# KatiaJDL/CenterPoly

Measured on AMD Instinct MI355X. Metric: inference img/s @2048x1024 DLA-34 (1 GPU), higher is better.
Workload: dtype f32 I/O; split-bf16 x3 contraction (a*b ~ ah*bh + ah*bl + al*bh on bf16 MFMA, ~2^-16 per product) in the convolutions, the heads and DCNv2; f32 accumulate; 1 GPU; BASELINE config 2: DLA-34 + DCNv2, 1x3x1024x2048 synthetic, 16-vertex cartesian head, K=128, forward + sigmoid + NMS/top-k/decode; parallelism=single

## Files before the change

### centerpoly_amd/_C.py

```python
import ctypes
import os
from ctypes import POINTER, Structure, c_char_p, c_float, c_int32, c_int64, c_size_t, c_void_p

import torch

_HERE = os.path.dirname(os.path.abspath(__file__))
LIB_PATH = os.path.join(_HERE, "csrc", "libcenterpoly_hip.so")

CP_OK = 0
REP = {"cartesian": 0, "polar": 1, "polar_fixed": 2}
HEATMAP_UMICH, HEATMAP_ELLIPSE = 0, 1
L1_PLAIN, L1_POLAR, L1_POLAR_FIXED, L1_RELU20, L1_SMOOTH = 0, 1, 2, 3, 4
DCN_BWD_EXACT_F32, DCN_BWD_NARROW_TILES = 1, 2
DCN_CONTRACTION = {"f32": 0, "bf16x3": 1, "bf16x3_region": 3}


class DcnShape(Structure):
    _fields_ = [(n, c_int32) for n in ("B", "Cin", "H", "W", "Cout", "kh", "kw", "stride", "pad",
                                       "dil", "deformable_groups")]


class TargetShape(Structure):
    _fields_ = [(n, c_int32) for n in ("B", "max_objs", "nbr_points", "num_classes", "out_h", "out_w",
                                       "rep", "no_reorder_flip")]
# ... 62 lines not shown
                                        c_size_t, _P]),
    "cp_polygon_masks_workspace_bytes": (c_size_t, [c_int32, c_int32]),
    "cp_polygon_masks": (c_int32, [_P, _P, c_int32, c_int32, c_int32, _P, _P, _P, c_size_t, _P]),
    "cp_annot_rays_ids": (c_int32, [_P, c_int32, c_int32, _P, _P, c_int32, c_int32, _P, _P]),
    "cp_annot_rays_masks": (c_int32, [_P, c_int32, c_int32, _P, c_int32, c_int32, _P, _P]),
    "cp_polygon_paint_workspace_bytes": (c_size_t, [c_int32, c_int32]),
    "cp_polygon_paint": (c_int32, [_P, _P, _P, c_int32, c_int32, c_int32, c_int32, _P, _P, c_size_t, _P]),
    "cp_render_overlay_workspace_bytes": (c_size_t, [c_int32, c_int32]),
    "cp_render_overlay": (c_int32, [_P, c_int32, c_int32, _P, c_int32, c_int32, _P, _P, _P, _P, c_int32, _P, c_int32, _P,
                                    c_int32, _P, _P, _P, c_size_t, _P]),
    "cp_render_heatmap": (c_int32, [_P, c_int32, c_int32, c_int32, c_int32, _P, _P, _P, _P, c_int32, c_int32, _P, _P]),
    "cp_oracle_map": (c_int32, [_P, _P] + [c_int32] * 5 + [_P, _P]),
    "cp_id_histogram": (c_int32, [_P, c_int32, c_int32, _P, _P]),
    "cp_instance_overlaps_workspace_bytes": (c_size_t, [c_int32] * 4),
    "cp_instance_overlaps": (c_int32, [_P, c_int32, _P, c_int32, c_int32, _P, c_int32, _P, c_int32, _P, _P, _P, _P,
                                       c_size_t, _P]),
    "cp_polydet_post_process": (c_int32, [_P, _P, c_float, c_int32, c_int32, c_int32, _P, _P]),
    "cp_polydet_targets_workspace_bytes": (c_size_t, [POINTER(TargetShape)]),
    "cp_polydet_targets": (c_int32, [POINTER(TargetShape)] + [_P] * 19 + [_P, c_size_t, _P]),
    "cp_polydet_targets_ex": (c_int32, [POINTER(TargetShape), c_int32] + [_P] * 19 + [_P, c_size_t, _P]),
    "cp_polydet_dense_targets": (c_int32, [POINTER(TargetShape), _P, _P, c_size_t, _P, _P, _P]),
    "cp_conv_direct_supported": (c_int32, [c_int32] * 5),
    "cp_conv_direct_wgrad_supported": (c_int32, [c_int32] * 5),
    "cp_conv_direct_wgrad": (c_int32, [_P, _P, _P] + [c_int32] * 8 + [_P]),
    "cp_conv_direct_forward": (c_int32, [_P, _P, _P, _P] + [c_int32] * 9 + [_P]),
    "cp_conv_direct_forward_ex": (c_int32, [_P, _P, _P, _P] + [c_int32] * 10 + [_P]),
    "cp_conv3x3_mfma_supported": (c_int32, [c_int32] * 4),
    "cp_conv3x3_mfma_weight_bytes": (c_size_t, [c_int32] * 2),
    "cp_conv3x3_mfma_prepare": (c_int32, [_P, c_int32, c_int32, c_int32, _P, _P]),
    "cp_conv3x3_mfma_forward": (c_int32, [_P, _P, _P, _P, _P] + [c_int32] * 6 + [_P]),
    "cp_conv_mfma_weight_bytes": (c_size_t, [c_int32] * 3),
    "cp_conv_mfma_prepare": (c_int32, [_P, c_int32, c_int32, c_int32, c_int32, _P, _P]),
    "cp_conv3x3_s2_wgrad_supported": (c_int32, [c_int32] * 4),
    "cp_conv3x3_s2_wgrad": (c_int32, [_P, _P, _P] + [c_int32] * 5 + [_P]),
    "cp_conv7x7_c3_supported": (c_int32, [c_int32] * 4),
    "cp_conv7x7_c3_weight_bytes": (c_size_t, [c_int32]),
    "cp_conv7x7_c3_prepare": (c_int32, [_P, c_int32, _P, _P]),
    "cp_conv7x7_c3_forward": (c_int32, [_P, _P, _P, _P] + [c_int32] * 6 + [_P]),
    "cp_conv_mfma_prepare_blocks": (c_int32, [c_int32] * 3),
    "cp_conv_mfma_prepare_batch": (c_int32, [_P, c_int32, c_int32, _P]),
    "cp_conv_mfma_forward": (c_int32, [_P, _P, c_int32, _P, _P, _P, _P] + [c_int32] * 6 + [_P]),
    "cp_conv_mfma_forward_strided": (c_int32, [_P, _P, c_int32, _P, _P, _P, _P] + [c_int32] * 7 + [_P]),
    "cp_dla_base_pair_supported": (c_int32, [c_int32] * 2),
    "cp_dla_base_pair_forward": (c_int32, [_P] * 6 + [c_int32] * 3 + [_P]),
    "cp_conv_mfma_forward_split": (c_int32, [_P, c_int32, _P, _P, _P, _P] + [c_int32] * 9 + [_P]),
    "cp_activation_split": (c_int32, [_P, _P] + [c_int32] * 4 + [_P]),
    "cp_activation_unsplit": (c_int32, [_P, _P] + [c_int32] * 4 + [_P]),
    "cp_conv1x1_stream_supported": (c_int32, [_P, c_int32, c_int32, c_int32, c_int32]),
    "cp_conv1x1_stream_weight_bytes": (c_size_t, [c_int32] * 2),
    "cp_conv1x1_stream_prepare": (c_int32, [_P, c_int32, c_int32, _P, _P]),
    "cp_conv1x1_stream_forward": (c_int32, [_P, _P, c_int32, _P, _P, _P, _P] + [c_int32] * 5 + [_P]),
    "cp_conv1x1_stream_form": (c_int32, [c_int32] * 5),
    "cp_conv1x1_stream_forward_form": (c_int32, [_P, _P, c_int32, _P, _P, _P, _P] + [c_int32] * 7 + [_P]),
    "cp_conv_mfma_input_grad_relu_workspace_bytes": (c_size_t, [c_int32] * 4),
    "cp_conv_mfma_input_grad_relu": (c_int32, [_P] * 5 + [c_int32] * 6 + [_P, c_size_t, _P]),
    "cp_conv3x3_s2_input_grad": (c_int32, [_P, _P, _P, _P] + [c_int32] * 5 + [_P]),
    "cp_conv3x3_mfma_wgrad_supported": (c_int32, [c_int32] * 4),
    "cp_conv3x3_mfma_wgrad": (c_int32, [_P, _P, _P] + [c_int32] * 5 + [_P]),
    "cp_conv_mfma_wgrad": (c_int32, [_P, _P, _P] + [c_int32] * 6 + [_P]),
    "cp_heads_fused_w2_bytes": (c_size_t, [c_int32]),
    "cp_heads_fused_prepare_w2": (c_int32, [_P, c_int32, c_int32, _P, _P]),
    "cp_heads_fused_forward": (c_int32, [_P, _P, _P, _P, _P, _P, _P] + [c_int32] * 6 + [_P]),
    "cp_maxpool2x2_forward": (c_int32, [_P, _P] + [c_int32] * 4 + [_P]),
    "cp_maxpool2x2_backward": (c_int32, [_P, _P, _P] + [c_int32] * 4 + [_P]),
    "cp_conv1x1_act_forward": (c_int32, [_P, c_int64, _P, c_int32, _P, _P, _P, c_int32, c_int32, c_int32, c_int64, _P]),
    "cp_soft_nms": (c_int32, [_P, c_int32, c_int32, c_float, c_float, c_float, c_int32]),
    "cp_soft_nms_device": (c_int32, [_P, c_int32, _P, _P, c_int32, c_float, c_float, c_float, c_int32, _P, _P]),
    "cp_merge_detections_workspace_bytes": (c_size_t, [c_int32] * 4),
    "cp_merge_detections": (c_int32, [_P] + [c_int32] * 6 + [c_float] * 3 + [c_int32, _P, _P, _P, c_size_t, _P]),
    "cp_polydet_decode_workspace_bytes": (c_size_t, [c_int32] * 5),
    "cp_polydet_decode": (c_int32, [_P, _P, _P, _P] + [c_int32] * 7 + [_P, _P, _P, _P, c_size_t, _P]),
    "cp_polydet_decode_ex": (c_int32, [_P, _P, _P, _P] + [c_int32] * 8 + [_P, _P, _P, _P, c_size_t, _P]),
    "cp_sigmoid_focal_workspace_bytes": (c_size_t, [c_int64]),
    "cp_sigmoid_focal_forward": (c_int32, [_P, _P, c_int64, _P, _P, _P, c_size_t, _P]),
    "cp_sigmoid_focal_backward": (c_int32, [_P, _P, c_int64, _P, _P, _P, _P]),
    "cp_gather_l1_forward": (c_int32, [_P, _P, _P, _P, _P] + [c_int32] * 6 + [c_float, _P, _P]),
    "cp_gather_l1_backward": (c_int32, [_P, _P, _P, _P, _P] + [c_int32] * 6 + [c_float, _P, _P, _P]),
    "cp_mse_workspace_bytes": (c_size_t, []),
    "cp_mse_forward": (c_int32, [_P, _P, c_int64, _P, _P, c_size_t, _P]),
    "cp_mse_backward": (c_int32, [_P, _P, c_int64, _P, _P, _P]),
    "cp_dense_l1_workspace_bytes": (c_size_t, []),
    "cp_dense_l1_forward": (c_int32, [_P, _P, _P, c_int64, c_float, _P, _P, c_size_t, _P]),
    "cp_dense_l1_backward": (c_int32, [_P, _P, _P, c_int64, _P, _P, _P, _P]),
    "cp_poly_iou_order_workspace_bytes": (c_size_t, [c_int32] * 3),
    "cp_poly_iou_order_forward": (c_int32, [_P, _P, _P, _P] + [c_int32] * 6 + [_P, _P, _P, _P,
                                                                               c_size_t, _P]),
    "cp_poly_iou_order_backward": (c_int32, [_P, _P, _P, _P] + [c_int32] * 6 + [_P, _P, _P, _P,
                                                                                c_size_t, _P]),
}

EXPORTS = tuple(_SIGNATURES)


def lib():
    global _lib
    if _lib is None:
        if not os.path.exists(LIB_PATH):
            raise NativeLibraryMissing(
                "%s not found: build it with `python -c 'import __graft_entry__ as g; g.build()'` "
                "(or `make -C centerpoly_amd/csrc`). centerpoly_amd has no CPU fallback." % LIB_PATH)
        l = ctypes.CDLL(LIB_PATH)
        for name, (res, args) in _SIGNATURES.items():
            fn = getattr(l, name)
            fn.restype = res
            fn.argtypes = args
        if l.cp_abi_version() != ABI_VERSION:
# ... 103 lines not shown
```

### centerpoly_amd/models/networks/conv3x3.py

```python

import weakref

import torch
import torch.nn.functional as F

from ... import _C
from .prepared import prepared

_ENABLED = True
_WGRAD = True
MIN_CIN = 24
MIN_WORKGROUPS = 128
STREAM_1X1 = "auto"


def _workgroups(B, cout, H, W):
    return B * ((W + 31) // 32) * ((H + 3) // 4) * ((cout + 31) // 32)


def _fills(B, cin, cout, H, W):
    n = _workgroups(B, cout, H, W)
    return n >= MIN_WORKGROUPS or (cin >= 256 and n >= 16)


def usable_shape(x, cout):
    if not (_ENABLED and x.is_cuda and x.dtype == torch.float32 and x.dim() == 4):
        return False
    B, cin, H, W = x.shape
    return cin >= MIN_CIN and bool(_C.lib().cp_conv3x3_mfma_supported(cin, cout, H, W)) \
        and _fills(B, cin, cout, H, W)


def usable(conv, x):
    k = conv.kernel_size
    if not (k in ((3, 3), (1, 1)) and conv.padding == (k[0] // 2, k[0] // 2) and conv.dilation == (1, 1)
            and conv.groups == 1 and conv.padding_mode == "zeros"):
        return False
    if conv.stride == (1, 1):
        return usable_shape(x, conv.out_channels)
    if conv.stride == (2, 2) and k == (3, 3) and x.dim() == 4:
        B, cin, H, W = x.shape
        return usable_shape(x, conv.out_channels) and _fills(B, cin, conv.out_channels, (H - 1) // 2 + 1, (W - 1) // 2 + 1)
    return False


class _WeightBank(object):

    def __init__(self):
        self.entries = {}
        self.table = None

    def get(self, weight, cin, cout, code):
        if not isinstance(weight, torch.nn.Parameter):
            return None
        key = (id(weight), cin, cout, code)
        e = self.entries.get(key)
        if e is None or e[0]() is not weight:
            self.entries[key] = [weakref.ref(weight), None, -1, weight.data_ptr(), weight.device]
            self.table = None
            return None
        if e[1] is None or e[2] != weight._version or e[3] != weight.data_ptr() or e[4] != weight.device:
            return None
        return e[1]

    def refresh(self):
        L = _C.lib()
# ... 52 lines not shown

def _permute(weight, cin, cout, code):
    L = _C.lib()
    taps = weight.shape[2] * weight.shape[3]
    wp = torch.empty(L.cp_conv_mfma_weight_bytes(cin, cout, taps), dtype=torch.uint8, device=weight.device)
    _C.check(L.cp_conv_mfma_prepare(_C.ptr(weight), cin, cout, taps, code, _C.ptr(wp), _C.stream()), "cp_conv_mfma_prepare")
    return wp


def _launch(x, wp, bias, residual, cout, relu, taps=9, stride=1):
    B, cin, H, W = x.shape
    out = torch.empty((B, cout, (H - 1) // stride + 1, (W - 1) // stride + 1), dtype=torch.float32, device=x.device)
    tag = ("conv3x3_fwd" if stride == 1 else "conv3x3s2_fwd") if taps == 9 else "conv1x1_fwd"
    end = _C.kernel_timer.start((tag, cin, cout, H, W, B)) if _C.kernel_timer is not None else None
    ptrs, chans = (_C.c_void_p * 1)(x.data_ptr()), (_C.c_int32 * 1)(cin)
    _C.check(_C.lib().cp_conv_mfma_forward_strided(ptrs, chans, 1, _C.ptr(wp), _C.ptr(bias), _C.ptr(residual),
                                                   _C.ptr(out), B, H, W, cout, taps, stride, 1 if relu else 0,
                                                   _C.stream()), "cp_conv_mfma_forward_strided")
    if end is not None:
        end.record()
    return out


def _stream_wins(cin, cout, H, W):
    return (cin, cout, H * W) in _STREAM_SHAPES


_STREAM_SHAPES = frozenset([(256, 128, 128 * 256), (448, 128, 128 * 256), (512, 256, 64 * 128), (896, 256, 64 * 128),
                            (1280, 512, 32 * 64)])


def _stream_infer(xs, cs, owner, w, bias, residual, relu, slot):
    x0 = xs[0]
    B, _, H, W = x0.shape
    cin, cout, n = sum(cs), w.shape[0], len(xs)
    if not (STREAM_1X1 == "force" or _stream_wins(cin, cout, H, W)) or B > 65535:
        return None
    L = _C.lib()
    chans = (_C.c_int32 * n)(*cs)
    if not L.cp_conv1x1_stream_supported(chans, n, cout, H, W):
        return None
    wp, _ = prepared(owner, slot, (w,), lambda: _permute(w.contiguous(), cin, cout, 0))
    xs = [x.contiguous() for x in xs]
    out = torch.empty((B, cout, H, W), dtype=torch.float32, device=x0.device)
    ptrs = (_C.c_void_p * n)(*[x.data_ptr() for x in xs])
    end = _C.kernel_timer.start(("conv1x1_fwd", cin, cout, H, W, B)) if _C.kernel_timer is not None else None
    _C.check(L.cp_conv1x1_stream_forward(ptrs, chans, n, _C.ptr(wp), _C.ptr(bias), _C.ptr(residual), _C.ptr(out), B, H, W,
                                         cout, 1 if relu else 0, _C.stream()), "cp_conv1x1_stream_forward")
    if end is not None:
        end.record()
    return out


def conv_infer(xs, owner, w, bias=None, residual=None, relu=False, conv=None, slot="conv", x_split=False,
               out_split=False):
    k = tuple(w.shape[2:])
    if not _ENABLED or k not in ((1, 1), (3, 3)):
        return None
    if (x_split or out_split) and (len(xs) != 1 or k != (3, 3) or (out_split and residual is not None)
                                   or (x_split and xs[0].shape[1] % 32) or (out_split and w.shape[0] % 8)):
        return None
    stride = 1
    if conv is not None:
        if not (conv.stride in ((1, 1), (2, 2)) and conv.padding == (k[0] // 2, k[0] // 2)
                and conv.dilation == (1, 1) and conv.groups == 1 and conv.padding_mode == "zeros"):
            return None
        stride = conv.stride[0]
    x0 = xs[0]
    if not all(x.is_cuda and x.dtype == torch.float32 and x.dim() == 4 and x.shape[0] == x0.shape[0]
               and x.shape[2:] == x0.shape[2:] for x in xs) or len(xs) > 4:
        return None
    cs = [x.shape[1] for x in xs]
    cin, cout = sum(cs), w.shape[0]
    B, _, H, W = x0.shape
    Ho, Wo = (H - 1) // stride + 1, (W - 1) // stride + 1
    L = _C.lib()
    if k == (1, 1) and stride == 1 and STREAM_1X1 != "off" and not (x_split or out_split) and cin == w.shape[1] \
            and (residual is None or residual.is_contiguous()):
        out = _stream_infer(xs, cs, owner, w, bias, residual, relu, slot)
        if out is not None:
            return out
    if cin != w.shape[1] or cin < MIN_CIN or (len(xs) > 1 and any(c % 32 for c in cs)) \
            or not all(L.cp_conv3x3_mfma_supported(c, cout, H, W) for c in cs) \
            or not _fills(B, cin, cout, Ho, Wo) or (residual is not None and not residual.is_contiguous()):
        return None
    taps = k[0] * k[1]
    wp, _ = prepared(owner, slot, (w,), lambda: _permute(w.contiguous(), cin, cout, 0))
    xs = [x.contiguous() for x in xs]
    out = torch.empty((B, cout, Ho, Wo), dtype=torch.float32, device=x0.device)
    ptrs = (_C.c_void_p * len(xs))(*[x.data_ptr() for x in xs])
    chans = (_C.c_int32 * len(xs))(*cs)
    tag = "conv3x3_fwd" if taps == 9 and stride == 1 else ("conv3x3s2_fwd" if taps == 9 else "conv1x1_fwd")
    end = _C.kernel_timer.start((tag, cin, cout, H, W, B)) if _C.kernel_timer is not None else None
    if x_split or out_split:
        if x_split and stride != 1:
            return None
        _C.check(L.cp_conv_mfma_forward_split(_C.ptr(xs[0]), 1 if x_split else 0, _C.ptr(wp), _C.ptr(bias),
                                              _C.ptr(residual), _C.ptr(out), 1 if out_split else 0, B, cin, H, W, cout,
                                              taps, stride, 1 if relu else 0, _C.stream()), "cp_conv_mfma_forward_split")
    else:
        _C.check(L.cp_conv_mfma_forward_strided(ptrs, chans, len(xs), _C.ptr(wp), _C.ptr(bias), _C.ptr(residual),
                                                _C.ptr(out), B, H, W, cout, taps, stride, 1 if relu else 0, _C.stream()),
                 "cp_conv_mfma_forward_strided")
    if end is not None:
        end.record()
    return out


def block_infer(x, conv1, wb1, conv2, wb2, skip):
    planes = wb1[0].shape[0]
    if not (_ENABLED and x.is_cuda and planes % 32 == 0 and tuple(wb1[0].shape[2:]) == (3, 3)
            and tuple(wb2[0].shape[2:]) == (3, 3) and conv2.stride == (1, 1)):
        return None
    B, _, H, W = x.shape
    s = conv1.stride[0]
    Ho, Wo = (H - 1) // s + 1, (W - 1) // s + 1
    if planes < MIN_CIN or not _fills(B, planes, planes, Ho, Wo) \
            or not _C.lib().cp_conv3x3_mfma_supported(planes, planes, Ho, Wo) or (skip is not None and not skip.is_contiguous()):
        return None
    y = conv_infer([x], conv1, wb1[0], wb1[1], None, True, conv=conv1, out_split=True)
    if y is None:
        return None
    z = conv_infer([y], conv2, wb2[0], wb2[1], skip, True, conv=conv2, x_split=True)
    if z is None:
        raise _C.NativeError("block_infer: the second convolution refused a split tensor its first convolution wrote")
    return z


def s2_input_grad(xshape, weight, go):
    L = _C.lib()
    B, cin, H, W = xshape
    cout = weight.shape[0]
    Ho, Wo = (H - 1) // 2 + 1, (W - 1) // 2 + 1
    if not (_ENABLED and go.is_cuda and go.dtype == torch.float32 and tuple(weight.shape[2:]) == (3, 3)
            and tuple(go.shape) == (B, cout, Ho, Wo) and cout >= MIN_CIN and L.cp_conv3x3_mfma_supported(cout, cin, Ho, Wo)
            and cin * H * W * 4 < 0x7FFFFFF0 and _fills(B, cout, cin, Ho, Wo)):
        return None
    go = go.contiguous()
    gx = torch.empty(xshape, dtype=torch.float32, device=go.device)
# ... 316 lines not shown
```

### include/centerpoly_hip.h

```cpp
#ifndef CENTERPOLY_HIP_H
#define CENTERPOLY_HIP_H

#include <stddef.h>
#include <stdint.h>

#ifdef __cplusplus
extern "C" {
#endif

#define CP_ABI_VERSION 3

enum {
  CP_OK = 0,
  CP_EINVAL = -1,
  CP_EUNSUPPORTED = -2,
  CP_EWORKSPACE = -3,
  CP_EHIP = -4
};

enum { CP_REP_CARTESIAN = 0, CP_REP_POLAR = 1, CP_REP_POLAR_FIXED = 2 };

enum {
  CP_DCN_F32 = 0,
  CP_DCN_BF16X3 = 1,
// ... 77 lines not shown
int cp_bias_relu_backward(const float* y, const float* grad_out, float* grad_in, float* grad_bias,
                          int32_t B, int32_t C, int64_t HW, void* stream);
int cp_channel_sum_accumulate(const float* x, float* out, int32_t B, int32_t C, int64_t HW, void* stream);

int cp_conv_direct_supported(int32_t Cin, int32_t Cout, int32_t k, int32_t stride, int32_t pad);
int cp_conv_direct_forward(const float* x, const float* w, const float* bias, float* out, int32_t B, int32_t Cin,
                           int32_t H, int32_t W, int32_t Cout, int32_t k, int32_t stride, int32_t pad,
                           int32_t relu, void* stream);
int cp_conv_direct_forward_ex(const float* x, const float* w, const float* bias, float* out, int32_t B, int32_t Cin,
                           int32_t H, int32_t W, int32_t Cout, int32_t k, int32_t stride, int32_t pad,
                           int32_t relu, int32_t split_bf16, void* stream);

int cp_conv3x3_mfma_supported(int32_t Cin, int32_t Cout, int32_t H, int32_t W);
size_t cp_conv3x3_mfma_weight_bytes(int32_t Cin, int32_t Cout);
int cp_conv3x3_mfma_prepare(const float* weight, int32_t Cin, int32_t Cout, int32_t transposed, void* wperm,
                            void* stream);
int cp_conv3x3_mfma_forward(const float* x, const void* wperm, const float* bias, const float* residual, float* out,
                            int32_t B, int32_t Cin, int32_t H, int32_t W, int32_t Cout, int32_t relu, void* stream);

size_t cp_conv_mfma_weight_bytes(int32_t Cin, int32_t Cout, int32_t taps);
int cp_conv_mfma_prepare(const float* weight, int32_t Cin, int32_t Cout, int32_t taps, int32_t transposed, void* wperm,
                         void* stream);
typedef struct cp_conv_prepare_job {
  const float* weight;
  void* wperm;
  int32_t Cin, Cout, taps, transposed, first_block, reserved;
} cp_conv_prepare_job;
int32_t cp_conv_mfma_prepare_blocks(int32_t Cin, int32_t Cout, int32_t taps);
int cp_conv_mfma_prepare_batch(const cp_conv_prepare_job* jobs_device, int32_t njobs, int32_t total_blocks, void* stream);
int cp_conv_mfma_forward(const float* const* xs, const int32_t* cs, int32_t nsrc, const void* wperm, const float* bias,
                         const float* residual, float* out, int32_t B, int32_t H, int32_t W, int32_t Cout,
                         int32_t taps, int32_t relu, void* stream);
int cp_conv_mfma_forward_strided(const float* const* xs, const int32_t* cs, int32_t nsrc, const void* wperm,
                                 const float* bias, const float* residual, float* out, int32_t B, int32_t H, int32_t W,
                                 int32_t Cout, int32_t taps, int32_t stride, int32_t relu, void* stream);
int cp_dla_base_pair_supported(int32_t H, int32_t W);
int cp_dla_base_pair_forward(const float* x, const float* w0, const float* b0, const float* w1, const float* b1, float* out,
                             int32_t B, int32_t H, int32_t W, void* stream);
int cp_conv_mfma_forward_split(const void* x, int32_t x_split, const void* wperm, const float* bias, const float* residual,
                               void* out, int32_t out_split, int32_t B, int32_t Cin, int32_t H, int32_t W, int32_t Cout,
                               int32_t taps, int32_t stride, int32_t relu, void* stream);
int cp_activation_split(const float* x, void* out, int32_t B, int32_t C, int32_t H, int32_t W, void* stream);
int cp_activation_unsplit(const void* in, float* x, int32_t B, int32_t C, int32_t H, int32_t W, void* stream);
int cp_conv1x1_stream_supported(const int32_t* cs, int32_t nsrc, int32_t Cout, int32_t H, int32_t W);
size_t cp_conv1x1_stream_weight_bytes(int32_t Cin, int32_t Cout);
int cp_conv1x1_stream_prepare(const float* weight, int32_t Cin, int32_t Cout, void* wperm, void* stream);
int cp_conv1x1_stream_forward(const float* const* xs, const int32_t* cs, int32_t nsrc, const void* wperm, const float* bias,
                              const float* residual, float* out, int32_t B, int32_t H, int32_t W, int32_t Cout,
                              int32_t relu, void* stream);
int cp_conv1x1_stream_form(int32_t Cin, int32_t Cout, int32_t H, int32_t W, int32_t B);
int cp_conv1x1_stream_forward_form(const float* const* xs, const int32_t* cs, int32_t nsrc, const void* wperm,
                                   const float* bias, const float* residual, float* out, int32_t B, int32_t H, int32_t W,
                                   int32_t Cout, int32_t relu, int32_t nb, int32_t ks, void* stream);
int cp_conv3x3_s2_wgrad_supported(int32_t Cin, int32_t Cout, int32_t H, int32_t W);
int cp_conv3x3_s2_wgrad(const float* x, const float* grad_out, float* gw, int32_t B, int32_t Cin, int32_t H, int32_t W,
                        int32_t Cout, void* stream);

int cp_conv7x7_c3_supported(int32_t Cout, int32_t H, int32_t W, int32_t stride);
size_t cp_conv7x7_c3_weight_bytes(int32_t Cout);
int cp_conv7x7_c3_prepare(const float* weight, int32_t Cout, void* wperm, void* stream);
int cp_conv7x7_c3_forward(const float* x, const void* wperm, const float* bias, float* out, int32_t B, int32_t H,
                          int32_t W, int32_t Cout, int32_t stride, int32_t relu, void* stream);

size_t cp_conv_mfma_input_grad_relu_workspace_bytes(int32_t B, int32_t Cin, int32_t H, int32_t W);
int cp_conv_mfma_input_grad_relu(const float* grad_out, const void* wperm_t, const float* y, float* grad_y,
                                 float* grad_bias, int32_t B, int32_t Cin, int32_t H, int32_t W, int32_t Cout,
                                 int32_t taps, void* workspace, size_t workspace_bytes, void* stream);
int cp_conv3x3_s2_input_grad(const float* grad_out, const void* wperm_t, const float* residual, float* grad_in, int32_t B,
                             int32_t Cin, int32_t H, int32_t W, int32_t Cout, void* stream);

int cp_conv3x3_mfma_wgrad_supported(int32_t Cin, int32_t Cout, int32_t H, int32_t W);
int cp_conv3x3_mfma_wgrad(const float* x, const float* go, float* gw, int32_t B, int32_t Cin, int32_t H, int32_t W,
                          int32_t Cout, void* stream);
int cp_conv_mfma_wgrad(const float* x, const float* go, float* gw, int32_t B, int32_t Cin, int32_t H, int32_t W,
                       int32_t Cout, int32_t taps, void* stream);

int cp_conv_direct_wgrad_supported(int32_t Cin, int32_t Cout, int32_t k, int32_t stride, int32_t pad);
int cp_conv_direct_wgrad(const float* x, const float* go, float* gw, int32_t B, int32_t Cin, int32_t H, int32_t W,
                         int32_t Cout, int32_t k, int32_t stride, int32_t pad, void* stream);

size_t cp_heads_fused_w2_bytes(int32_t head_conv);
int cp_heads_fused_prepare_w2(const float* w2, int32_t cout, int32_t head_conv, void* w2perm, void* stream);
int cp_heads_fused_forward(const float* x, const void* wperm1, const float* b1, const void* const* w2perm,
                           const float* const* b2, float* const* out, const int32_t* cout, int32_t nheads, int32_t B,
                           int32_t Cin, int32_t H, int32_t W, int32_t head_conv, void* stream);

int cp_conv1x1_act_forward(const float* y, int64_t y_bstride, const float* in_bias, int32_t relu_in,
                           const float* w_t, const float* bias, float* out, int32_t B, int32_t Cin,
                           int32_t Cout, int64_t HW, void* stream);

int cp_instance_masks(const int32_t* poly, const uint8_t* flags, int32_t n, int32_t N, int32_t H, int32_t W,
                      uint8_t* masks, int32_t* counts, void* stream);

int cp_id_histogram(const uint16_t* ids, int32_t H, int32_t W, int32_t* hist, void* stream);
size_t cp_instance_overlaps_workspace_bytes(int32_t n, int32_t G, int32_t H, int32_t W);
int cp_instance_overlaps(const uint8_t* masks, int32_t n, const uint16_t* gt_ids, int32_t H, int32_t W,
                         const int32_t* inst_ids, int32_t G, const int32_t* void_ids, int32_t V, int32_t* inter,
                         int32_t* void_inter, int32_t* pred_pixels, void* workspace, size_t workspace_bytes,
                         void* stream);

int cp_writer_instances(const float* rows, int32_t R, int32_t N, float thresh, const int32_t* class_table, int32_t C,
                        int32_t* n_out, int32_t* src, int32_t* poly, uint8_t* flags, int32_t* label, float* conf,
                        void* stream);

int cp_class_instance_masks(const int32_t* poly, const int32_t* group, const uint8_t* flags, int32_t n, int32_t N,
                            int32_t H, int32_t W, uint8_t* masks, int32_t* counts, void* stream);
// ... 165 lines not shown
```

Before: 379.5 img/s.

## Add streaming 3x3 conv kernel for narrow-output DCN offset convolutions

Adds a new HIP kernel for 3x3 stride-1 convolutions with at most 32 output channels. It streams input straight from global memory into registers via buffer loads, splits values into bf16 hi/lo on the fly and runs bf16x3 MFMA, with optional split-K across waves reduced through LDS. A row4 variant loads 64-pixel rows once and builds the left/right tap shifts with DPP lane moves, so input reuse across taps replaces reloading. The path is enabled only for three hard-coded (Cin, Cout=27, HW) shapes, which look like the DCNv2 offset/mask convs at this resolution. It adds kernel variants and shape-specific dispatch.

```diff
diff --git a/centerpoly_amd/_C.py b/centerpoly_amd/_C.py
--- a/centerpoly_amd/_C.py
+++ b/centerpoly_amd/_C.py
@@ -138,6 +138,10 @@
     "cp_conv1x1_stream_forward": (c_int32, [_P, _P, c_int32, _P, _P, _P, _P] + [c_int32] * 5 + [_P]),
     "cp_conv1x1_stream_form": (c_int32, [c_int32] * 5),
     "cp_conv1x1_stream_forward_form": (c_int32, [_P, _P, c_int32, _P, _P, _P, _P] + [c_int32] * 7 + [_P]),
+    "cp_conv3x3_stream_supported": (c_int32, [c_int32] * 4),
+    "cp_conv3x3_stream_form": (c_int32, [c_int32] * 5),
+    "cp_conv3x3_stream_forward": (c_int32, [_P] * 5 + [c_int32] * 6 + [_P]),
+    "cp_conv3x3_stream_forward_form": (c_int32, [_P] * 5 + [c_int32] * 8 + [_P]),
     "cp_conv_mfma_input_grad_relu_workspace_bytes": (c_size_t, [c_int32] * 4),
     "cp_conv_mfma_input_grad_relu": (c_int32, [_P] * 5 + [c_int32] * 6 + [_P, c_size_t, _P]),
     "cp_conv3x3_s2_input_grad": (c_int32, [_P, _P, _P, _P] + [c_int32] * 5 + [_P]),
diff --git a/centerpoly_amd/csrc/conv3x3_stream.hip b/centerpoly_amd/csrc/conv3x3_stream.hip
--- /dev/null
+++ b/centerpoly_amd/csrc/conv3x3_stream.hip
@@ -0,0 +1,426 @@
+#include <type_traits>
+
+#include "cp_common.h"
+
+namespace {
+
+typedef __bf16 bf16x8 __attribute__((ext_vector_type(8)));
+typedef __bf16 bf16x2 __attribute__((ext_vector_type(2)));
+typedef float f32x2 __attribute__((ext_vector_type(2)));
+typedef unsigned u32x4 __attribute__((ext_vector_type(4)));
+
+constexpr int KC = 32;
+constexpr int TAPS = 9;
+constexpr int MT = 2;
+constexpr unsigned OOB = 0x80000000u;
+
+constexpr int DEPTH_TAP = 2;
+
+struct Stream3Args {
+  const float* x;
+  const bf16x8* wp;
+  const float* bias;
+  float* out;
+  int Cin, Cout, H, W, nchunk, tpr, ntiles, vec;
+  int tpr4, ntiles4;
+};
+
+__device__ __forceinline__ void split2(float v0, float v1, unsigned& hi, unsigned& lo) {
+  const bf16x2 h = __builtin_convertvector(f32x2{v0, v1}, bf16x2);
+  const unsigned hb = __builtin_bit_cast(unsigned, h);
+  const float h0 = __builtin_bit_cast(float, hb << 16), h1 = __builtin_bit_cast(float, hb & 0xffff0000u);
+  const bf16x2 l = __builtin_convertvector(f32x2{v0 - h0, v1 - h1}, bf16x2);
+  hi = hb;
+  lo = __builtin_bit_cast(unsigned, l);
+}
+
+template <int NT, int KS>
+__global__ __launch_bounds__(256, 2) void conv3x3_stream_kernel(Stream3Args a) {
+  constexpr int PG = 4 / KS, DEPTH = DEPTH_TAP;
+  const int lane = threadIdx.x & 63;
+  const int wave = __builtin_amdgcn_readfirstlane(threadIdx.x >> 6);
+  const int q = wave % KS, grp = wave / KS;
+  const int c = lane & 15, g = lane >> 4;
+  int lw = blockIdx.x;
+  if ((gridDim.x & 7) == 0) lw = (blockIdx.x & 7) * (gridDim.x >> 3) + (blockIdx.x >> 3);
+  const int T0 = (lw * PG + grp) * NT, b = blockIdx.y;
+  const int W = a.W, H = a.H, HW = H * W;
+  const unsigned plane = (unsigned)HW * 4u;
+
+  int ty[NT];
+  unsigned vin[NT], edge[NT];
+#pragma unroll
+  for (int n = 0; n < NT; ++n) {
+    const int T = T0 + n;
+    ty[n] = T < a.ntiles ? T / a.tpr : -4;
+    const int x = (T % a.tpr) * 16 + c;
+    edge[n] = x >= W ? 7u : (x == 0 ? 1u : 0u) | (x == W - 1 ? 4u : 0u);
+    vin[n] = ((unsigned)(8 * g) * (unsigned)HW + (unsigned)(ty[n] * W + x)) * 4u;
+  }
+
+  const unsigned tbytes = (unsigned)a.nchunk * TAPS * 2048u, wlane = (unsigned)lane * 16u;
+  const __amdgpu_buffer_rsrc_t rs_w =
+      __builtin_amdgcn_make_buffer_rsrc(const_cast<bf16x8*>(a.wp), 0, (int)(MT * tbytes), 0x00020000);
+  const int nmine = a.nchunk > q ? (a.nchunk - q + KS - 1) / KS : 0;
+  const int nsteps = nmine * TAPS;
+  const __amdgpu_buffer_rsrc_t rs_x = __builtin_amdgcn_make_buffer_rsrc(
+      const_cast<float*>(a.x + (long long)b * a.Cin * HW), 0, (int)((unsigned)a.Cin * plane), 0x00020000);
+
+  int ic = 0, it = 0;
+  auto issue_x = [&](float (&v)[NT][8]) __attribute__((always_inline)) {
+    const bool live = ic < nmine;
+    const int dy = (it * 11) >> 5, dx = it - 3 * dy;
+    const unsigned delta = (unsigned)(((dy - 1) * W + (dx - 1)) * 4);
+    const unsigned cbase = (unsigned)(live ? (q + ic * KS) * KC : 0) * plane;
+#pragma unroll
+    for (int n = 0; n < NT; ++n) {
+      const int yy = ty[n] + dy - 1;
+      const bool rowok = live && yy >= 0 && yy < H;
+      const unsigned bad = rowok ? (edge[n] >> dx) & 1u : 1u;
+      const unsigned vo = bad ? OOB : vin[n] + delta;
+#pragma unroll
+      for (int j = 0; j < 8; ++j)
+        v[n][j] = __builtin_bit_cast(float, __builtin_amdgcn_raw_buffer_load_b32(rs_x, vo + (cbase + (unsigned)j * plane), 0, 0));
+    }
+  };
+  auto issue_w = [&](bf16x8 (&w)[MT][2]) __attribute__((always_inline)) {
+    const unsigned wo = ic < nmine ? wlane + (unsigned)((q + ic * KS) * TAPS + it) * 2048u : OOB;
+#pragma unroll
+    for (int m = 0; m < MT; ++m) {
+      w[m][0] = __builtin_bit_cast(bf16x8, __builtin_amdgcn_raw_buffer_load_b128(rs_w, wo + (unsigned)m * tbytes, 0, 0));
+      w[m][1] = __builtin_bit_cast(bf16x8, __builtin_amdgcn_raw_buffer_load_b128(rs_w, wo + (unsigned)m * tbytes + 1024u, 0, 0));
+    }
+    const bool wrap = it == TAPS - 1;
+    it = wrap ? 0 : it + 1;
+    ic += wrap ? 1 : 0;
+  };
+
+  f32x4 acc[MT][NT];
+#pragma unroll
+  for (int m = 0; m < MT; ++m)
+#pragma unroll
+    for (int n = 0; n < NT; ++n) acc[m][n] = f32x4{0.f, 0.f, 0.f, 0.f};
+
+  float v[DEPTH][NT][8];
+  bf16x8 w[DEPTH][MT][2];
+#pragma unroll
+  for (int d = 0; d < DEPTH; ++d) {
+    issue_x(v[d]);
+    __builtin_amdgcn_sched_barrier(0);
+    issue_w(w[d]);
+    __builtin_amdgcn_sched_barrier(0);
+  }
+
+  for (int s = 0; s < nsteps; s += DEPTH) {
+#pragma unroll
+    for (int d = 0; d < DEPTH; ++d) {
+      bf16x8 xh[NT], xl[NT];
+#pragma unroll
+      for (int n = 0; n < NT; ++n) {
+        unsigned hi[4], lo[4];
+#pragma unroll
+        for (int j = 0; j < 4; ++j) split2(v[d][n][2 * j], v[d][n][2 * j + 1], hi[j], lo[j]);
+        xh[n] = __builtin_bit_cast(bf16x8, hi);
+        xl[n] = __builtin_bit_cast(bf16x8, lo);
+      }
+      issue_x(v[d]);
+      __builtin_amdgcn_sched_barrier(0);
+#pragma unroll
+      for (int m = 0; m < MT; ++m)
+#pragma unroll
+        for (int n = 0; n < NT; ++n) {
+          acc[m][n] = __builtin_amdgcn_mfma_f32_16x16x32_bf16(xh[n], w[d][m][0], acc[m][n], 0, 0, 0);
+          acc[m][n] = __builtin_amdgcn_mfma_f32_16x16x32_bf16(xl[n], w[d][m][0], acc[m][n], 0, 0, 0);
+          acc[m][n] = __builtin_amdgcn_mfma_f32_16x16x32_bf16(xh[n], w[d][m][1], acc[m][n], 0, 0, 0);
+        }
+      __builtin_amdgcn_sched_barrier(0);
+      issue_w(w[d]);
+    }
+  }
+
+  constexpr int NTILE = MT * NT;
+  const __amdgpu_buffer_rsrc_t rs_o = __builtin_amdgcn_make_buffer_rsrc(a.out + (long long)b * a.Cout * HW, 0,
+                                                                        (int)((unsigned)a.Cout * plane), 0x00020000);
+  const __amdgpu_buffer_rsrc_t rs_b =
+      __builtin_amdgcn_make_buffer_rsrc(const_cast<float*>(a.bias), 0, a.bias ? a.Cout * 4 : 0, 0x00020000);
+  __shared__ f32x4 red[KS > 1 ? 4 * NTILE * 64 : 1];
+  if constexpr (KS > 1) {
+#pragma unroll
+    for (int m = 0; m < MT; ++m)
+#pragma unroll
+      for (int n = 0; n < NT; ++n) red[(wave * NTILE + m * NT + n) * 64 + lane] = acc[m][n];
+    __syncthreads();
+  }
+#pragma unroll
+  for (int m = 0; m < MT; ++m) {
+    const int co = m * 16 + c;
+    const float bv = __builtin_bit_cast(float, __builtin_amdgcn_raw_buffer_load_b32(rs_b, (unsigned)co * 4u, 0, 0));
+#pragma unroll
+    for (int n = 0; n < NT; ++n) {
+      const int t = m * NT + n;
+      if (KS > 1 && t % KS != q) continue;
+      f32x4 s = acc[m][n];
+      if constexpr (KS > 1) {
+        s = red[((grp * KS + 0) * NTILE + t) * 64 + lane];
+#pragma unroll
+        for (int k = 1; k < KS; ++k) s += red[((grp * KS + k) * NTILE + t) * 64 + lane];
+      }
+      f32x4 o;
+#pragma unroll
+      for (int r = 0; r < 4; ++r) o[r] = s[r] + bv;
+      const int T = T0 + n, x = (T % a.tpr) * 16 + 4 * g;
+      const bool ok = T < a.ntiles && co < a.Cout;
+      const unsigned off = ((unsigned)co * (unsigned)HW + (unsigned)(ty[n] * W + x)) * 4u;
+      if (a.vec) {
+        __builtin_amdgcn_raw_buffer_store_b128(__builtin_bit_cast(u32x4, o), rs_o, ok && x < W ? off : OOB, 0, 0);
+      } else {
+#pragma unroll
+        for (int r = 0; r < 4; ++r)
+          __builtin_amdgcn_raw_buffer_store_b32(__builtin_bit_cast(unsigned, (float)o[r]), rs_o,
+                                                ok && x + r < W ? off + 4u * r : OOB, 0, 0);
+      }
+    }
+  }
+}
+
+__device__ __forceinline__ unsigned row_from_left(unsigned old, unsigned src) {
+  return (unsigned)__builtin_amdgcn_update_dpp((int)old, (int)src, 0x111, 0xF, 0xF, false);
+}
+__device__ __forceinline__ unsigned row_from_right(unsigned old, unsigned src) {
+  return (unsigned)__builtin_amdgcn_update_dpp((int)old, (int)src, 0x101, 0xF, 0xF, false);
+}
+
+template <int KS>
+__global__ __launch_bounds__(256, 2) void conv3x3_stream_row4_kernel(Stream3Args a) {
+  constexpr int PG = 4 / KS, NT = 4, NTILE = MT * NT;
+  const int lane = threadIdx.x & 63;
+  const int wave = __builtin_amdgcn_readfirstlane(threadIdx.x >> 6);
+  const int q = wave % KS, grp = wave / KS;
+  const int c = lane & 15, g = lane >> 4;
+  int lw = blockIdx.x;
+  if ((gridDim.x & 7) == 0) lw = (blockIdx.x & 7) * (gridDim.x >> 3) + (blockIdx.x >> 3);
+  const int T = lw * PG + grp, b = blockIdx.y;
+  const int W = a.W, H = a.H, HW = H * W;
+  const unsigned plane = (unsigned)HW * 4u;
+  const int ty = T < a.ntiles4 ? T / a.tpr4 : -4;
+  const int X0 = (T % a.tpr4) * 64, x = X0 + 4 * c;
+  const int hx = c == 0 ? X0 - 1 : c == 15 ? X0 + 64 : -1;
+  const unsigned vin = x < W ? ((unsigned)(8 * g) * (unsigned)HW + (unsigned)(ty * W + x)) * 4u : OOB;
+  const unsigned hin = hx >= 0 && hx < W ? ((unsigned)(8 * g) * (unsigned)HW + (unsigned)(ty * W + hx)) * 4u : OOB;
+
+  const unsigned tbytes = (unsigned)a.nchunk * TAPS * 2048u, wlane = (unsigned)lane * 16u;
+  const __amdgpu_buffer_rsrc_t rs_w =
+      __builtin_amdgcn_make_buffer_rsrc(const_cast<bf16x8*>(a.wp), 0, (int)(MT * tbytes), 0x00020000);
+  const int nmine = a.nchunk > q ? (a.nchunk - q + KS - 1) / KS : 0;
+  const int nsteps = nmine * 3;
+  const __amdgpu_buffer_rsrc_t rs_x = __builtin_amdgcn_make_buffer_rsrc(
+      const_cast<float*>(a.x + (long long)b * a.Cin * HW), 0, (int)((unsigned)a.Cin * plane), 0x00020000);
+
+  int ic = 0, ir = 0;
+  auto issue_x = [&](f32x4 (&cv)[8], float (&hv)[8]) __attribute__((always_inline)) {
+    const bool live = ic < nmine;
+    const int yy = ty + ir - 1;
+    const bool rowok = live && yy >= 0 && yy < H;
+    const unsigned rdelta = (unsigned)((ir - 1) * W * 4);
+    const unsigned cbase = (unsigned)(live ? (q + ic * KS) * KC : 0) * plane;
+    const unsigned vo = rowok ? vin + rdelta : OOB, ho = rowok ? hin + rdelta : OOB;
+#pragma unroll
+    for (int j = 0; j < 8; ++j) {
+      cv[j] = __builtin_bit_cast(f32x4, __builtin_amdgcn_raw_buffer_load_b128(rs_x, vo + (cbase + (unsigned)j * plane), 0, 0));
+      hv[j] = __builtin_bit_cast(float, __builtin_amdgcn_raw_buffer_load_b32(rs_x, ho + (cbase + (unsigned)j * plane), 0, 0));
+    }
+  };
+  auto issue_w = [&](int t, bf16x8 (&w)[MT][2]) __attribute__((always_inline)) {
+    const unsigned wo = ic < nmine ? wlane + (unsigned)((q + ic * KS) * TAPS + 3 * ir + t) * 2048u : OOB;
+#pragma unroll
+    for (int m = 0; m < MT; ++m) {
+      w[m][0] = __builtin_bit_cast(bf16x8, __builtin_amdgcn_raw_buffer_load_b128(rs_w, wo + (unsigned)m * tbytes, 0, 0));
+      w[m][1] = __builtin_bit_cast(bf16x8, __builtin_amdgcn_raw_buffer_load_b128(rs_w, wo + (unsigned)m * tbytes + 1024u, 0, 0));
+    }
+  };
+  auto next_step = [&]() __attribute__((always_inline)) {
+    const bool wrap = ir == 2;
+    ir = wrap ? 0 : ir + 1;
+    ic += wrap ? 1 : 0;
+  };
+
+  f32x4 acc[MT][NT];
+#pragma unroll
+  for (int m = 0; m < MT; ++m)
+#pragma unroll
+    for (int e = 0; e < NT; ++e) acc[m][e] = f32x4{0.f, 0.f, 0.f, 0.f};
+
+  f32x4 cv[8];
+  float hv[8];
+  bf16x8 w[3][MT][2];
+  issue_x(cv, hv);
+  __builtin_amdgcn_sched_barrier(0);
+#pragma unroll
+  for (int t = 0; t < 3; ++t) issue_w(t, w[t]);
+  next_step();
+  __builtin_amdgcn_sched_barrier(0);
+
+  for (int s = 0; s < nsteps; ++s) {
+    unsigned ch[NT][4], cl[NT][4], hh[4], hl[4];
+#pragma unroll
+    for (int k = 0; k < 4; ++k) {
+#pragma unroll
+      for (int e = 0; e < NT; ++e) split2(cv[2 * k][e], cv[2 * k + 1][e], ch[e][k], cl[e][k]);
+      split2(hv[2 * k], hv[2 * k + 1], hh[k], hl[k]);
+    }
+    issue_x(cv, hv);
+    __builtin_amdgcn_sched_barrier(0);
+    unsigned lh[4], ll[4], rh[4], rl[4];
+#pragma unroll
+    for (int k = 0; k < 4; ++k) {
+      lh[k] = row_from_left(hh[k], ch[3][k]);
+      ll[k] = row_from_left(hl[k], cl[3][k]);
+      rh[k] = row_from_right(hh[k], ch[0][k]);
+      rl[k] = row_from_right(hl[k], cl[0][k]);
+    }
+#pragma unroll
+    for (int t = 0; t < 3; ++t) {
+#pragma unroll
+      for (int m = 0; m < MT; ++m)
+#pragma unroll
+        for (int e = 0; e < NT; ++e) {
+          const unsigned(&ph)[4] = t == 1 ? ch[e] : t == 0 ? (e == 0 ? lh : ch[e == 0 ? 0 : e - 1]) : (e == 3 ? rh : ch[e == 3 ? 3 : e + 1]);
+          const unsigned(&pl)[4] = t == 1 ? cl[e] : t == 0 ? (e == 0 ? ll : cl[e == 0 ? 0 : e - 1]) : (e == 3 ? rl : cl[e == 3 ? 3 : e + 1]);
+          const bf16x8 xh = __builtin_bit_cast(bf16x8, ph), xl = __builtin_bit_cast(bf16x8, pl);
+          acc[m][e] = __builtin_amdgcn_mfma_f32_16x16x32_bf16(xh, w[t][m][0], acc[m][e], 0, 0, 0);
+          acc[m][e] = __builtin_amdgcn_mfma_f32_16x16x32_bf16(xl, w[t][m][0], acc[m][e], 0, 0, 0);
+          acc[m][e] = __builtin_amdgcn_mfma_f32_16x16x32_bf16(xh, w[t][m][1], acc[m][e], 0, 0, 0);
+        }
+      __builtin_amdgcn_sched_barrier(0);
+      issue_w(t, w[t]);
+      __builtin_amdgcn_sched_barrier(0);
+    }
+    next_step();
+  }
+
+  const __amdgpu_buffer_rsrc_t rs_o = __builtin_amdgcn_make_buffer_rsrc(a.out + (long long)b * a.Cout * HW, 0,
+                                                                        (int)((unsigned)a.Cout * plane), 0x00020000);
+  const __amdgpu_buffer_rsrc_t rs_b =
+      __builtin_amdgcn_make_buffer_rsrc(const_cast<float*>(a.bias), 0, a.bias ? a.Cout * 4 : 0, 0x00020000);
+  __shared__ f32x4 red[KS > 1 ? 4 * NTILE * 64 : 1];
+  if constexpr (KS > 1) {
+#pragma unroll
+    for (int m = 0; m < MT; ++m)
+#pragma unroll
+      for (int e = 0; e < NT; ++e) red[(wave * NTILE + m * NT + e) * 64 + lane] = acc[m][e];
+    __syncthreads();
+  }
+#pragma unroll
+  for (int m = 0; m < MT; ++m) {
+    const int co = m * 16 + c;
+    const float bv = __builtin_bit_cast(float, __builtin_amdgcn_raw_buffer_load_b32(rs_b, (unsigned)co * 4u, 0, 0));
+#pragma unroll
+    for (int r = 0; r < 4; ++r) {
+      if (KS > 1 && (m * 4 + r) % KS != q) continue;
+      f32x4 o;
+#pragma unroll
+      for (int e = 0; e < NT; ++e) {
+        float sum = acc[m][e][r];
+        if constexpr (KS > 1) {
+          sum = red[((grp * KS + 0) * NTILE + m * NT + e) * 64 + lane][r];
+#pragma unroll
+          for (int k = 1; k < KS; ++k) sum += red[((grp * KS + k) * NTILE + m * NT + e) * 64 + lane][r];
+        }
+        o[e] = sum + bv;
+      }
+      const int xo = X0 + 16 * g + 4 * r;
+      const bool ok = T < a.ntiles4 && co < a.Cout && xo < W;
+      const unsigned off = ((unsigned)co * (unsigned)HW + (unsigned)(ty * W + xo)) * 4u;
+      __builtin_amdgcn_raw_buffer_store_b128(__builtin_bit_cast(u32x4, o), rs_o, ok ? off : OOB, 0, 0);
+    }
+  }
+}
+
+int staged_ks(int Cin, int Cout, int H, int W, int B) {
+  const int nchunk = (Cin + KC - 1) / KC;
+  const long long tiles_x = (W + 31) / 32;
+  auto wgs = [&](int mt, int th) { return tiles_x * ((H + th - 1) / th) * B * ((Cout + 16 * mt - 1) / (16 * mt)); };
+  if (wgs(2, 16) >= 448) return 1;
+  if (wgs(2, 8) >= 320) return 1;
+  if (wgs(2, 4) < 384 && nchunk >= 8) return 4;
+  if (wgs(2, 4) < 768 && nchunk >= 4) return 2;
+  return 1;
+}
+
+int pick_nt(int H, int W) {
+  if ((long long)H * W < 8192) return 1;
+  return (W & 3) == 0 ? 4 : 2;
+}
+
+bool shape_ok(int Cin, int Cout, int H, int W) {
+  if (Cin < 1 || Cout < 1 || Cout > 16 * MT || H < 1 || W < 1) return false;
+  const long long HW = (long long)H * W;
+  if ((Cin + 2ll * KC) * HW * 4 >= (1ll << 31) || Cin >= (1 << 20)) return false;
+  return true;
+}
+
+}
+
+int cp_conv3x3_stream_supported(int32_t Cin, int32_t Cout, int32_t H, int32_t W) { return shape_ok(Cin, Cout, H, W) ? 1 : 0; }
+
+int cp_conv3x3_stream_form(int32_t Cin, int32_t Cout, int32_t H, int32_t W, int32_t B) {
+  return pick_nt(H, W) << 8 | staged_ks(Cin, Cout, H, W, B);
+}
+
+int cp_conv3x3_stream_forward_form(const float* x, const void* wperm, const float* bias, const float* residual, float* out,
+                                   int32_t B, int32_t Cin, int32_t H, int32_t W, int32_t Cout, int32_t relu, int32_t nt,
+                                   int32_t ks, void* stream) {
+  CP_CHECK_ARG(x && wperm && out && B >= 1 && Cin >= 1 && H >= 1 && W >= 1 && Cout >= 1);
+  if (!shape_ok(Cin, Cout, H, W) || B > 65535 || residual || relu) return CP_EUNSUPPORTED;
+  Stream3Args a;
+  a.x = x;
+  a.wp = (const bf16x8*)wperm;
+  a.bias = bias;
+  a.out = out;
+  a.Cin = Cin;
+  a.Cout = Cout;
+  a.H = H;
+  a.W = W;
+  a.nchunk = (Cin + KC - 1) / KC;
+  a.tpr = (W + 15) / 16;
+  a.ntiles = H * a.tpr;
+  a.vec = (W & 3) == 0 && (reinterpret_cast<unsigned long long>(out) & 15) == 0;
+  a.tpr4 = (W + 63) / 64;
+  a.ntiles4 = H * a.tpr4;
+  if (nt == 0 && ks == 0) {
+    nt = pick_nt(H, W);
+    ks = staged_ks(Cin, Cout, H, W, B);
+  }
+  if ((nt != 1 && nt != 2 && nt != 4) || (ks != 1 && ks != 2 && ks != 4)) return CP_EINVAL;
+  const auto launch = [&](auto kernel) {
+    const unsigned npg = (unsigned)((a.ntiles + nt - 1) / nt), pgw = 4 / ks;
+    hipLaunchKernelGGL(kernel, dim3((npg + pgw - 1) / pgw, B), dim3(256), 0, (hipStream_t)stream, a);
+  };
+  if (nt == 4 && a.vec) {
+    const auto launch4 = [&](auto kernel) {
+      const unsigned pgw = 4 / ks;
+      hipLaunchKernelGGL(kernel, dim3(((unsigned)a.ntiles4 + pgw - 1) / pgw, B), dim3(256), 0, (hipStream_t)stream, a);
+    };
+    if (ks == 1) launch4(conv3x3_stream_row4_kernel<1>);
+    else if (ks == 2) launch4(conv3x3_stream_row4_kernel<2>);
+    else launch4(conv3x3_stream_row4_kernel<4>);
+  } else if (nt == 4) {
+    if (ks == 1) launch(conv3x3_stream_kernel<4, 1>);
+    else if (ks == 2) launch(conv3x3_stream_kernel<4, 2>);
+    else launch(conv3x3_stream_kernel<4, 4>);
+  } else if (nt == 2) {
+    if (ks == 1) launch(conv3x3_stream_kernel<2, 1>);
+    else if (ks == 2) launch(conv3x3_stream_kernel<2, 2>);
+    else launch(conv3x3_stream_kernel<2, 4>);
+  } else {
+    if (ks == 1) launch(conv3x3_stream_kernel<1, 1>);
+    else if (ks == 2) launch(conv3x3_stream_kernel<1, 2>);
+    else launch(conv3x3_stream_kernel<1, 4>);
+  }
+  return cp_launch_status();
+}
+
+int cp_conv3x3_stream_forward(const float* x, const void* wperm, const float* bias, const float* residual, float* out,
+                              int32_t B, int32_t Cin, int32_t H, int32_t W, int32_t Cout, int32_t relu, void* stream) {
+  return cp_conv3x3_stream_forward_form(x, wperm, bias, residual, out, B, Cin, H, W, Cout, relu, 0, 0, stream);
+}
diff --git a/centerpoly_amd/models/networks/conv3x3.py b/centerpoly_amd/models/networks/conv3x3.py
--- a/centerpoly_amd/models/networks/conv3x3.py
+++ b/centerpoly_amd/models/networks/conv3x3.py
@@ -12,6 +12,7 @@
 MIN_CIN = 24
 MIN_WORKGROUPS = 128
 STREAM_1X1 = "auto"
+STREAM_3X3 = "auto"
 
 
 def _workgroups(B, cout, H, W):
@@ -170,6 +171,32 @@
     return out
 
 
+def _stream3_wins(cin, cout, H, W):
+    return (cin, cout, H * W) in _STREAM3_SHAPES
+
+
+_STREAM3_SHAPES = frozenset([(128, 27, 128 * 256), (256, 27, 64 * 128), (512, 27, 32 * 64)])
+
+
+def _stream3_infer(x, owner, w, bias, slot):
+    B, cin, H, W = x.shape
+    cout = w.shape[0]
+    if not (STREAM_3X3 == "force" or _stream3_wins(cin, cout, H, W)) or B > 65535:
+        return None
+    L = _C.lib()
+    if not L.cp_conv3x3_stream_supported(cin, cout, H, W):
+        return None
+    wp, _ = prepared(owner, slot, (w,), lambda: _permute(w.contiguous(), cin, cout, 0))
+    x = x.contiguous()
+    out = torch.empty((B, cout, H, W), dtype=torch.float32, device=x.device)
+    end = _C.kernel_timer.start(("conv3x3_fwd", cin, cout, H, W, B)) if _C.kernel_timer is not None else None
+    _C.check(L.cp_conv3x3_stream_forward(_C.ptr(x), _C.ptr(wp), _C.ptr(bias), None, _C.ptr(out), B, cin, H, W, cout, 0,
+                                         _C.stream()), "cp_conv3x3_stream_forward")
+    if end is not None:
+        end.record()
+    return out
+
+
 def conv_infer(xs, owner, w, bias=None, residual=None, relu=False, conv=None, slot="conv", x_split=False,
                out_split=False):
     k = tuple(w.shape[2:])
@@ -203,6 +230,11 @@
             or not _fills(B, cin, cout, Ho, Wo) or (residual is not None and not residual.is_contiguous()):
         return None
     taps = k[0] * k[1]
+    if k == (3, 3) and stride == 1 and len(xs) == 1 and cout <= 32 and residual is None and not relu \
+            and not (x_split or out_split) and STREAM_3X3 != "off":
+        out = _stream3_infer(x0, owner, w, bias, slot)
+        if out is not None:
+            return out
     wp, _ = prepared(owner, slot, (w,), lambda: _permute(w.contiguous(), cin, cout, 0))
     xs = [x.contiguous() for x in xs]
     out = torch.empty((B, cout, Ho, Wo), dtype=torch.float32, device=x0.device)
diff --git a/include/centerpoly_hip.h b/include/centerpoly_hip.h
--- a/include/centerpoly_hip.h
+++ b/include/centerpoly_hip.h
@@ -153,6 +153,13 @@
 int cp_conv1x1_stream_forward_form(const float* const* xs, const int32_t* cs, int32_t nsrc, const void* wperm,
                                    const float* bias, const float* residual, float* out, int32_t B, int32_t H, int32_t W,
                                    int32_t Cout, int32_t relu, int32_t nb, int32_t ks, void* stream);
+int cp_conv3x3_stream_supported(int32_t Cin, int32_t Cout, int32_t H, int32_t W);
+int cp_conv3x3_stream_form(int32_t Cin, int32_t Cout, int32_t H, int32_t W, int32_t B);
+int cp_conv3x3_stream_forward(const float* x, const void* wperm, const float* bias, const float* residual, float* out,
+                              int32_t B, int32_t Cin, int32_t H, int32_t W, int32_t Cout, int32_t relu, void* stream);
+int cp_conv3x3_stream_forward_form(const float* x, const void* wperm, const float* bias, const float* residual, float* out,
+                                   int32_t B, int32_t Cin, int32_t H, int32_t W, int32_t Cout, int32_t relu, int32_t nt,
+                                   int32_t ks, void* stream);
 int cp_conv3x3_s2_wgrad_supported(int32_t Cin, int32_t Cout, int32_t H, int32_t W);
 int cp_conv3x3_s2_wgrad(const float* x, const float* grad_out, float* gw, int32_t B, int32_t Cin, int32_t H, int32_t W,
                         int32_t Cout, void* stream);
```

Measured after the change: 392.9 img/s, median of 6. 3.5% higher.
